# Naxaes/Rust-Swift-Raytracer

Measured on AMD Instinct MI355X. Metric: Mrays/sec + frames/sec at 1920×1080 spp=64; 1/2/4/8 MI355X, higher is better.
Workload: dtype f32; 1 GPU; c2: 1920x1080, spp 64, depth 8, 486 spheres, 0 triangles, COUNTER RNG; width=1920, height=1080, spp=64, depth=8, parallelism=one device renders the frame in place (no RCCL call)

## Files before the change

rust-swift-raytracer_amd/csrc/render.h:

```cpp
#pragma once

#include <hip/hip_runtime.h>

#include <cstdint>

#include "fastdiv.h"

namespace rtamd {

enum : uint32_t { kRngCounter = 1, kRngReplay = 2 };
enum : uint32_t { kRngSerialCount = 3, kRngSerialEstimate = 4, kRngSerialCheck = 5, kRngSerialCoalesce = 6,
                  kRngSerialPixel = 7 };
enum : uint32_t { kMatDiffuse = 0, kMatMetal = 1, kMatDielectric = 2, kMatEmission = 3 };
constexpr uint32_t kPrimaryTriStripW = 8;
#ifndef RT_TRACE_RING
#define RT_TRACE_RING 4
#endif
constexpr uint32_t kTraceRing = RT_TRACE_RING;
#ifdef RT_STAMPS
constexpr uint32_t kStatSlots = 24;
#else
constexpr uint32_t kStatSlots = 16;
#endif
constexpr uint32_t kStampSegs = 8;

struct SerialPred {
    const double *P;
    const double *mu;
    uint32_t spp, npix;
};
RT_HOST_DEVICE inline double serial_M(const SerialPred &m, uint32_t j) {
    const uint32_t p = j / m.spp;
    return p < m.npix ? m.P[p] + (double)(j - p * m.spp) * m.mu[p] : m.P[m.npix];
}

constexpr uint32_t kMaxJobParts = 1024;

struct TraceParams {
    const float4 *sph_hot;
    const float4 *sph_cold;
    const float4 *tri_hot;
    const float4 *tri_geo;
    const float *mats;
    float *samples;
    float *ring;
    uint32_t ring_shift;
    uint32_t *out;
    float inv_spp;
    uint32_t alpha_u8;
    uint32_t *job_counter;
    uint32_t *job_counter_next;
    unsigned long long *stats;
    const uint32_t *replay;
    float cam[12];
    float wden, hden;
    float wrcp, hrcp;
    uint32_t xdiv_uv;
    uint32_t nsph, nsph_padded, ntri;
    uint32_t width, height, spp;
    int32_t depth;
    uint32_t mode, seed;
    uint32_t row_block, rank, nranks;
    uint32_t slab_row0;
    uint32_t njobs;
    uint32_t npix;
    uint32_t chunk;
    uint32_t nparts;
    const float4 *bvh_nodes;
    const uint32_t *bvh_miss;
    const uint16_t *bvh_miss16;
    const float4 *bvh_prims;
    const uint32_t *bvh_prim_id;
    const float4 *big_hot;
    const uint32_t *big_id;
    uint32_t nnodes, nbig, nprims;
    uint32_t use_lds;
    uint32_t ablate;
    const float4 *sph_shade;
    const uint32_t *sph_kind;
    FastDiv div_spp, div_width, div_rowblock;
    uint32_t refill_min;
    uint32_t walk_min;
    uint32_t tri_walk_min;
    uint32_t steps;
    uint32_t step;
    float bvh_c[3], bvh_r, bvh_rmax, bvh_mag, bvh_inv_rmin;
    const uint4 *tbvh_nodes;
    const float4 *tbvh_tris;
    const uint32_t *tbvh_loose;
    uint32_t tnodes, ttris, tloose;
    float tbvh_c[3], tbvh_r, tbvh_mag;
    float tbvh_oc[3];
    float tq_base[3], tq_step[3], tq_nbase, tq_nstep;
    const uint4 *tw_nodes;
    uint32_t tw_depth;
    uint32_t wsteps;
    float cq_base[3], cq_step[3];
    const uint4 *cam_nodes;
    const float4 *cam_tris;
    uint32_t cam_nnodes;
    const uint32_t *ptl_off;
    const uint32_t *ptl_items;
    uint32_t ptl_spr;
    uint32_t ptl_always, ptl_end;
    const uint2 *spl;
    const uint32_t *win;
    SerialPred sM;
    const uint32_t *slo;
    const uint32_t *ctrl;
    uint32_t cbase;
    uint32_t nserial;
    uint32_t sspp;
    FastDiv div_sspp;
    uint32_t max_draws;
    uint32_t sL, sK;
    uint32_t gj32, gj_c0, gj_2p;
    const float4 *tw_tris;
    uint32_t tw_stride, tc_ncells;
    uint32_t tc_n[3];
    float tc_lo[3], tc_size, tc_inv_size;
    const uint4 *spix;
};

RT_HOST_DEVICE inline uint32_t serial_lo(const SerialPred &M, uint32_t a, uint32_t jl, uint32_t K,
                                         uint32_t depth, uint32_t nserial) {
    const uint32_t j = a + jl < nserial ? a + jl : nserial;
    double c = __builtin_floor(serial_M(M, j) - serial_M(M, a)) - (double)(K / 2u);
    const double hi = (double)depth * (double)jl;
    c = c < 0.0 ? 0.0 : c;
    c = c > hi ? hi : c;
    return (uint32_t)c;
}

hipError_t launch_trace(const TraceParams &p, uint32_t blocks, hipStream_t stream,
                        const uint4 *corner = nullptr);
hipError_t launch_sphere_lists(const float4 *prims, uint32_t n, const double *Mi, const double *o,
                               double e_abs, double wden, double hden, uint32_t width, uint32_t height,
                               int4 *rects, uint32_t *flag, uint2 *rec, hipStream_t stream);
size_t serial_tab_doubles(uint32_t npix);
hipError_t launch_serial_check_count(const float *flags, uint32_t n, unsigned long long *count,
                                     hipStream_t stream);
hipError_t launch_serial_moments(const float *est, uint32_t pix0, uint32_t n, uint32_t spp, uint32_t R,
                                 double scale, double *tab, uint32_t npix, hipStream_t stream);
hipError_t launch_serial_tables(double *tab, double *scratch, uint32_t npix, uint32_t spp, uint32_t L,
                                uint32_t n0, hipStream_t stream);
// ... 58 lines not shown
```

rust-swift-raytracer_amd/csrc/render.hip:

```cpp
#include <hip/hip_runtime.h>

#include <cstdint>
#include <type_traits>

#include "exactdiv.h"
#include "render.h"

#pragma clang fp contract(off)

namespace rtamd {
namespace {

struct F3 { float x, y, z; };

__device__ __forceinline__ F3 f3(float x, float y, float z) { return F3{x, y, z}; }
__device__ __forceinline__ F3 operator+(F3 a, F3 b) { return F3{a.x + b.x, a.y + b.y, a.z + b.z}; }
__device__ __forceinline__ F3 operator-(F3 a, F3 b) { return F3{a.x - b.x, a.y - b.y, a.z - b.z}; }
__device__ __forceinline__ F3 operator-(F3 a) { return F3{-a.x, -a.y, -a.z}; }
__device__ __forceinline__ F3 scale(F3 a, float s) { return F3{a.x * s, a.y * s, a.z * s}; }
__device__ __forceinline__ float dot(F3 a, F3 b) { return (a.x * b.x + a.y * b.y) + a.z * b.z; }
__device__ __forceinline__ F3 cross(F3 a, F3 b) {
    return F3{a.y * b.z - a.z * b.y, -(a.x * b.z - a.z * b.x), a.x * b.y - a.y * b.x};
}
__device__ __forceinline__ F3 divide_by(F3 a, float b) {
// ... 73 lines not shown
    return base[i];
#endif
}

__device__ __forceinline__ uint4 uniform_load_u4(const uint4 *base, uint32_t i) {
#if defined(__HIP_DEVICE_COMPILE__)
    typedef const __attribute__((address_space(4))) uint32_t *cu32_ptr;
    const cu32_ptr q = (cu32_ptr)(const void *)base + 4u * i;
    return make_uint4(q[0], q[1], q[2], q[3]);
#else
    return base[i];
#endif
}

__device__ __forceinline__ uint32_t fdiv(uint32_t n, const FastDiv &f) { return fastdiv_apply(n, f); }

constexpr uint32_t kWave = 64;
constexpr uint32_t kNodeEndDev = 0xFFFFFFFFu;
constexpr uint32_t kLeafBitDev = 0x80000000u;
constexpr uint32_t kSphListWalk = 0xFFFFu;
constexpr uint32_t kSphListMaxDev = 3u;
constexpr uint32_t kBatch = 8;

__device__ __forceinline__ void spheres_brute(const TraceParams &p, F3 org, F3 dir, float &best_t,
                                              int &best_i) {
    const float tmin = 0.001f;
#ifdef RT_BRUTE_PADDED
    const uint32_t n = p.nsph_padded;
#else
    const uint32_t n = p.nsph;
#endif
    for (uint32_t i0 = 0; i0 < n; i0 += kBatch) {
        const uint32_t m = n - i0;
        float hb[kBatch], disc[kBatch];
        bool any = false;
#pragma unroll
        for (uint32_t k = 0; k < kBatch; ++k) {
            hb[k] = 0.0f;
            disc[k] = -1.0f;
            if (k != 0u && k >= m) continue;
            const float4 S = uniform_load(p.sph_hot, i0 + k);
            const float ocx = org.x - S.x, ocy = org.y - S.y, ocz = org.z - S.z;
            hb[k] = (ocx * dir.x + ocy * dir.y) + ocz * dir.z;
            const float cc = ((ocx * ocx + ocy * ocy) + ocz * ocz) - S.w;
            disc[k] = hb[k] * hb[k] - cc;
            any |= disc[k] >= 0.0f;
        }
// ... 33 lines not shown
    const uint64_t kb = ((uint64_t)__float_as_uint(best_t) << 32) | (uint32_t)best_i;
    const bool take = valid && c != __builtin_inff() && kc < kb;
    if (take) { best_t = c; best_i = idx; }
    return take;
}

constexpr float kErrK = 3.0e-3f;

struct BvhView {
    const float4 *nodes;
    const uint32_t *miss32;
    const uint16_t *miss16;
    const float4 *prims;
    const uint32_t *ids;
    const float4 *shade;
    const uint32_t *kinds;
};

__device__ __forceinline__ float slab_rcp(float d) {
    return __builtin_amdgcn_fmed3f(__builtin_amdgcn_rcpf(d), -1e20f, 1e20f);
}

struct SphBound { float A, e_abs; };
__device__ __forceinline__ SphBound sph_bound(const TraceParams &p, F3 org) {
    const float ax = org.x - p.bvh_c[0], ay = org.y - p.bvh_c[1], az = org.z - p.bvh_c[2];
    return SphBound{__builtin_amdgcn_sqrtf((ax * ax + ay * ay) + az * az) * 1.00001f + p.bvh_r,
                    2e-6f * ((fabsf(org.x) + fabsf(org.y)) + fabsf(org.z) + p.bvh_mag)};
}
constexpr float kErrKq = 40.5f * 0x1p-24f;
__device__ __forceinline__ float sph_inflation(const TraceParams &p, SphBound b, float bt) {
    const float s = fminf(b.A, bt + p.bvh_rmax) * (1.0f + 3.0f * kErrK) + p.bvh_rmax;
    return fminf(kErrK * s, (kErrKq * s) * (s * p.bvh_inv_rmin)) + b.e_abs;
}

__device__ __forceinline__ void spheres_big(const TraceParams &p, F3 org, F3 dir, float &best_t,
                                            int &best_i) {
    for (uint32_t k = 0; k < p.nbig; ++k) {
        const float4 S = uniform_load(p.big_hot, k);
        sphere_candidate(S, org, dir, (int)uniform_load_u32(p.big_id, k), best_t, best_i);
    }
}

template <bool kLds>
__device__ __forceinline__ bool sphere_node(const BvhView &v, F3 inv, uint32_t ooff, float best_t, F3 nlo,
                                            F3 nhi, uint32_t &node, uint32_t &leaf, uint32_t &node_tests) {
    ++node_tests;
    float4 B0, B1;
    uint32_t miss, hit = 0;
    if (kLds) {
#if defined(__HIP_DEVICE_COMPILE__)
        typedef const __attribute__((address_space(3))) char *lds_cptr;
        const lds_cptr rec = (lds_cptr)(uintptr_t)node;
        B0 = *(const __attribute__((address_space(3))) float4 *)rec;
        B1 = *(const __attribute__((address_space(3))) float4 *)(rec + 16);
        const uint32_t lw = *(const __attribute__((address_space(3))) uint32_t *)(rec + 32 + ooff);
        hit = lw & 0xFFFFu;
        miss = lw >> 16;
#else
// ... 269 lines not shown
        const float omax = fmaxf(fmaxf(a, b), fmaxf(c, d));
        t0 = __builtin_fmaf(__builtin_fmaf(qlo, gs, omin), iv, c0);
        t1 = __builtin_fmaf(__builtin_fmaf(qhi, gs, omax), iv, c1);
    };
    float t0x, t1x, t0y, t1y, t0z, t1z;
    widen(lo16(w0), hi16(w1), nx0, nx1, nlo.x, nhi.x, gsx, inv.x, t0x, t1x);
    widen(hi16(w0), lo16(w2), ny0, ny1, nlo.y, nhi.y, gsy, inv.y, t0y, t1y);
    widen(lo16(w1), hi16(w2), nz0, nz1, nlo.z, nhi.z, gsz, inv.z, t0z, t1z);
    tn = fmaxf(fmaxf(fminf(t0x, t1x), fminf(t0y, t1y)), fminf(t0z, t1z));
    const float tf = fminf(fminf(fmaxf(t0x, t1x), fmaxf(t0y, t1y)), fmaxf(t0z, t1z));
    return !(tn > tf || tf < 0.001f || __float_as_int(tn) > __float_as_int(cap));
}

__device__ __forceinline__ void tri_leaf(const TraceParams &p, F3 org, F3 dir, bool cam,
                                         uint32_t leaf, float best_t, float &tri_t, int &tri_i,
                                         uint32_t &tri_in, uint32_t &tri_done, const float4 *wrecs = nullptr) {
    const float4 *recs = wrecs ? wrecs : cam ? p.cam_tris : p.tbvh_tris;
    const uint32_t first = leaf >> 3, end = first + (leaf & 7u);
    tri_done += leaf & 7u;
    for (uint32_t j = first; j < end; ++j)
        tri_record(recs + 4u * j, org, dir, best_t, tri_t, tri_i, tri_in);
}

template <bool kSerial>
__device__ __forceinline__ void job_pixel(const TraceParams &p, uint32_t job, uint32_t &s,
                                          uint32_t &col, uint32_t &row) {
    if (kSerial && p.mode == kRngSerialPixel) {
        const uint32_t pix = fdiv(p.cbase, p.div_sspp) + fdiv(job, p.div_spp);
        s = 0;
        row = fdiv(pix, p.div_width);
        col = pix - row * p.width;
        return;
    }
    if (kSerial) {
        const uint32_t jl = fdiv(job, p.div_spp);
        const uint32_t j = p.cbase + jl < p.nserial ? p.cbase + jl : p.nserial - 1u;
        const uint32_t pix = fdiv(j, p.div_sspp);
        s = j - pix * p.sspp;
        row = fdiv(pix, p.div_width);
        col = pix - row * p.width;
        return;
    }
    const uint32_t lp = fdiv(job, p.div_spp);
    s = job - lp * p.spp;
    const uint32_t q = fdiv(lp, p.div_width);
    col = lp - q * p.width;
    const uint32_t lr = p.slab_row0 + q;
    const uint32_t blk = fdiv(lr, p.div_rowblock);
    const uint32_t ir = (blk * p.nranks + p.rank) * p.row_block + (lr - blk * p.row_block);
    row = p.height - 1u - ir;
}

__device__ __forceinline__ void serial_pixel_span(const TraceParams &p, uint32_t q, uint32_t &plo,
                                                  uint32_t &phi) {
    if (p.spix != nullptr) {
        const uint4 s = p.spix[q];
        plo = s.x;
        phi = s.y;
        return;
    }
    const uint32_t a = p.cbase, ss = p.sspp;
    const uint32_t ln = min(p.sL, p.nserial - a);
    const uint32_t p0 = fdiv(a, p.div_sspp);
    const uint32_t jf = q == 0u ? 0u : (p0 + q) * ss - a;
    const uint32_t jz = min((p0 + q + 1u) * ss - a, ln) - 1u;
    plo = 2u * jf + 3u * p.slo[jf];
    phi = 2u * jz + 3u * (p.slo[jz] + p.sK - 1u);
}

__device__ __forceinline__ uint32_t serial_start(const TraceParams &p, uint32_t job) {
    const uint32_t jl = fdiv(job, p.div_spp);
    const uint32_t k = job - jl * p.spp;
    if (p.mode == kRngSerialCount)
// ... 11 lines not shown

__device__ __forceinline__ bool serial_pixel_job(const TraceParams &p, uint32_t job) {
    const uint32_t q = fdiv(job, p.div_spp);
    uint32_t plo, phi;
    serial_pixel_span(p, q, plo, phi);
    return plo + (job - q * p.spp) <= phi;
}

template <bool kSerial>
__device__ __forceinline__ void tri_primary_list(const TraceParams &p, uint32_t job, F3 org, F3 dir,
                                                 float best_t, float &tri_t, int &tri_i,
                                                 uint32_t &tri_in, uint32_t &tri_done) {
    uint32_t s, col, row;
    job_pixel<kSerial>(p, job, s, col, row);
    const uint32_t strip = row * p.ptl_spr + col / kPrimaryTriStripW;
    const uint32_t b = p.ptl_off[strip], e = p.ptl_off[strip + 1];
    tri_done += (e - b) + (p.ptl_end - p.ptl_always);
    for (uint32_t j = b; j < e; ++j)
        tri_record(p.cam_tris + 4u * p.ptl_items[j], org, dir, best_t, tri_t, tri_i, tri_in);
    for (uint32_t j = p.ptl_always; j < p.ptl_end; ++j)
        tri_record(p.cam_tris + 4u * p.ptl_items[j], org, dir, best_t, tri_t, tri_i, tri_in);
}

__device__ __forceinline__ uint32_t resolve_channel(const TraceParams &p, float sum) {
    return sat_u8(__builtin_sqrtf(sum * p.inv_spp) * 255.999f);
}
__device__ __forceinline__ void resolve_store_u8(const TraceParams &p, uint32_t lp, uint32_t R, uint32_t G,
                                                 uint32_t B) {
    const uint32_t q = fdiv(lp, p.div_width);
    const uint32_t col = lp - q * p.width;
    p.out[(size_t)(p.slab_row0 + q) * p.width + col] = R | (G << 8) | (B << 16) | (p.alpha_u8 << 24);
}
__device__ __forceinline__ void resolve_store(const TraceParams &p, uint32_t lp, float r, float g,
                                              float b) {
    resolve_store_u8(p, lp, resolve_channel(p, r), resolve_channel(p, g), resolve_channel(p, b));
}

#define RT_PLANE_LANES(mesh) ((mesh) < 2 || (mesh) == 3)
template <bool kPlaneLanes>
__device__ __forceinline__ void resolve_chunk(const TraceParams &p, const float *ring, uint32_t plane,
                                              uint32_t off, uint32_t base, uint32_t len,
                                              uint32_t lane) {
    __builtin_amdgcn_fence(__ATOMIC_RELEASE, "workgroup");
    __builtin_amdgcn_fence(__ATOMIC_ACQUIRE, "workgroup");
    const uint32_t spp = p.spp;
    const uint32_t np = fdiv(len, p.div_spp), pix0 = fdiv(base, p.div_spp);
    if (kPlaneLanes && 3u * np <= kWave && (spp & 3u) == 0) {
        const uint32_t c = lane >= np ? (lane >= 2u * np ? 2u : 1u) : 0u;
        const uint32_t g = lane - c * np;
        const bool on = lane < 3u * np;
        const float *src = ring + off + c * plane + (on ? g : 0u) * spp;
        float acc = 0.0f;
        for (uint32_t k = 0; k < spp; k += 16u) {
            float4 v[4];
#pragma unroll
            for (uint32_t q = 0; q < 4; ++q) {
                v[q] = make_float4(0.0f, 0.0f, 0.0f, 0.0f);
                if (on && k + 4u * q < spp) v[q] = *reinterpret_cast<const float4 *>(src + k + 4u * q);
            }
#pragma unroll
            for (uint32_t q = 0; q < 4; ++q) {
                if (k + 4u * q < spp) {
                    acc = acc + v[q].x;
                    acc = acc + v[q].y;
                    acc = acc + v[q].z;
                    acc = acc + v[q].w;
                }
            }
// ... 133 lines not shown
            const uint32_t ln = min(p.sL, p.nserial - p.cbase);
            const uint32_t p0 = fdiv(p.cbase, p.div_sspp);
            const uint32_t npq = E ? fdiv(p.cbase + ln - 1u, p.div_sspp) - p0 + 1u : 0u;
            p.spp = max(E, 1u);
            p.div_spp = make_fastdiv(p.spp);
            p.npix = npq;
            p.njobs = npq * E;
        }
    }
    if (!kSerial && p.job_counter_next != nullptr && blockIdx.x == 0)
        for (uint32_t i = threadIdx.x; i < kMaxJobParts; i += blockDim.x) p.job_counter_next[32u * i] = 0u;
    const uint32_t lane = __lane_id();
    auto kargs = [&]() -> const TraceParams & {
#if defined(__HIP_DEVICE_COMPILE__) && !defined(RT_NO_KARG_RELOAD)
        if (kSerial) return p;
        const __attribute__((address_space(4))) TraceParams *kp =
            (const __attribute__((address_space(4))) TraceParams *)__builtin_amdgcn_kernarg_segment_ptr();
        asm volatile("" : "+s"(kp));
        return *(const TraceParams *)kp;
#else
        return p;
#endif
    };
    extern __shared__ float4 lds[];
    BvhView view;
    const uint32_t sph_root = stage_tree<kLds, kCorner>(p, corner, lds, view);
    uint16_t *const tstack = reinterpret_cast<uint16_t *>(
                                 reinterpret_cast<char *>(lds) +
                                 (kLds ? (trace_tree_lds(p.nnodes, p.nprims, p.nsph_padded) + 15u) & ~(size_t)15u
                                       : 0u)) + threadIdx.x;
    uint32_t tsp = 0;

    F3 org = f3(0, 0, 0), dir = f3(0, 0, 0), inv = f3(0, 0, 0);
    float thr_r = 1.0f, thr_g = 1.0f, thr_b = 1.0f;
    uint32_t rng = 0, slot = ~0u, bounce = 0;
    uint32_t nscat = 0;
    uint32_t spl0 = 0, spl1 = kSphListWalk << 16;
    enum : uint32_t { kSetup = 0, kSph = 1, kTriInit = 2, kTri = 3, kShade = 4 };
    uint32_t phase = kSetup, node = 0, oct = 0;
    constexpr bool kWalkState = kMesh == 0 && !kStep;
    float best_t = 0.0f, tri_t = 0.0f, e = 0.0f;
    int best_i = -1, tri_i = -1;
    bool active = false;
    uint32_t rays = 0, tri_in = 0, sph_tests = 0, node_tests = 0, tnode_tests = 0,
             tri_done = 0;
    uint32_t it_all = 0, it_walk = 0, lanes_all = 0, lanes_walk = 0;
// ... 43 lines not shown
    } while (0)
#else
#define RT_STAMP(k) \
    do {            \
    } while (0)
#endif
    uint32_t part = (blockIdx.x * (blockDim.x / kWave) + threadIdx.x / kWave) % p.nparts;
    uint32_t tries = 0;
    auto part_begin = [&](uint32_t k) -> uint32_t {
        return (uint32_t)(((uint64_t)k * p.npix) / p.nparts) * p.spp;
    };
    uint32_t pbegin = part_begin(part), pend = part_begin(part + 1);
    uint32_t prefetch = 0;
    bool prefetch_pending = false;
    for (;;) {
        F3 vdir = dir;
        bool renorm = false;
        bool done = false;
        bool walked = false;
        const uint32_t nact = kCount ? (uint32_t)__popcll(__ballot(active)) : 0u;
        if (active) {
            float out_r = 0.0f, out_g = 0.0f, out_b = 0.0f;
            if (phase == kSetup) {
                const TraceParams &p = kargs();
                if ((int32_t)bounce >= p.depth) {
                    done = true;
                } else {
                    ++rays;
                    if (!kWalkState) {
                        inv = f3(slab_rcp(dir.x), slab_rcp(dir.y), slab_rcp(dir.z));
                        oct = (inv.x < 0.0f ? 1u : 0u) | (inv.y < 0.0f ? 2u : 0u) | (inv.z < 0.0f ? 4u : 0u);
                    }
                    best_t = __builtin_inff();
                    best_i = -1;
                    if (kBvh) {
                        spheres_big(p, org, dir, best_t, best_i);
                        if (!kWalkState)
                            node = kCorner ? sphere_corner_entry(sph_root, oct, p.nnodes)
                                           : sphere_walk_entry<kLds>(sph_root, oct, p.nnodes);
                        phase = (p.ablate & 1u) ? kTriInit : kSph;
                        if (!kMesh && bounce == 0 && (spl1 >> 16) != kSphListWalk) {
                            const uint32_t nc = spl1 >> 16;
                            sph_tests += nc;
                            if (nc > 0) sphere_candidate(view.prims[spl0 & 0xFFFFu], org, dir,
                                                         (int)view.ids[spl0 & 0xFFFFu], best_t, best_i);
                            if (nc > 1) sphere_candidate(view.prims[spl0 >> 16], org, dir,
                                                         (int)view.ids[spl0 >> 16], best_t, best_i);
                            if (nc > 2) sphere_candidate(view.prims[spl1 & 0xFFFFu], org, dir,
                                                         (int)view.ids[spl1 & 0xFFFFu], best_t, best_i);
                            phase = kTriInit;
                        }
                    } else {
                        spheres_brute(p, org, dir, best_t, best_i);
                        phase = kTriInit;
                    }
                }
            }
            RT_STAMP(1);
            uint32_t budget = p.steps;
            bool walk_now = true;
            if (!kMesh && p.walk_min != 0) {
                const uint32_t nwalk = (uint32_t)__popcll(__ballot(phase == kSph));
                const uint32_t nother = (uint32_t)__popcll(__ballot(phase != kSph && !done));
                walk_now = nwalk >= p.walk_min || nother == 0;
            }
            if (kBvh && phase == kSph && walk_now) {
                const TraceParams &p = kargs();
                walked = true;
                constexpr uint32_t kEnd = kLds ? 0xFFFFu : kNodeEndDev;
                const SphBound bnd = sph_bound(p, org);
                if (kWalkState) {
                    inv = f3(slab_rcp(dir.x), slab_rcp(dir.y), slab_rcp(dir.z));
                    oct = (inv.x < 0.0f ? 1u : 0u) | (inv.y < 0.0f ? 2u : 0u) | (inv.z < 0.0f ? 4u : 0u);
                    node = kCorner ? sphere_corner_entry(sph_root, oct, p.nnodes)
                                   : sphere_walk_entry<kLds>(sph_root, oct, p.nnodes);
                }
                if (kCorner) {
                    F3 nn, nf;
                    sphere_corner_slabs(org, inv, sph_inflation(p, bnd, best_t), oct, nn, nf);
                    const uint32_t offn = sph_root + 16u * oct, offf = sph_root + 112u - 16u * oct;
                    do {
                        uint32_t leaf;
                        if (sphere_node_corner(offn, offf, inv, best_t, nn, nf, node, leaf, node_tests))
                            sphere_leaf<true>(view, org, dir, leaf, best_t, best_i, sph_tests);
                    } while (node != 0xFFFFu && (!kStep || --budget != 0));
                } else {
                    F3 nlo, nhi;
                    sphere_slabs(org, inv, sph_inflation(p, bnd, best_t), nlo, nhi);
                    const uint32_t ooff = kLds ? 4u * oct : oct;
#ifdef RT_WALK_MIX
                    uint32_t wi = 0, wl = 0, wt = 0;
#endif
                    do {
                        uint32_t leaf;
                        const bool lf = sphere_node<kLds>(view, inv, ooff, best_t, nlo, nhi, node, leaf, node_tests);
#ifdef RT_WALK_MIX
                        if (kCount) {
                            ++wi;
// ... 260 lines not shown
            }
        }
        RT_STAMP(4);
        if (kCount && nact != 0) {
            const bool wk = __ballot(walked) != 0;
            ++it_all;
            lanes_all += nact;
            it_walk += wk ? 1u : 0u;
            lanes_walk += wk ? nact : 0u;
        }
        const uint64_t dead = __ballot(!active);
        const uint32_t ndead = (uint32_t)__popcll(dead);
        const bool refill = dead != 0 && (ndead >= p.refill_min || ndead == kWave);
        if (fused && refill) {
            const bool fin = !active && slot != ~0u;
            if (__ballot(fin) != 0) {
                const uint32_t lk = slot >> p.ring_shift;
#pragma unroll
                for (uint32_t k = 0; k < kTraceRing; ++k) {
                    if (rfree & (1u << k)) continue;
                    const uint32_t n = (uint32_t)__popcll(__ballot(fin && lk == k));
                    rleft[k] -= n;
                    if (n != 0 && rleft[k] == 0) {
                        const TraceParams &pc = kargs();
                        if (!(pc.ablate & 2u))
                            resolve_chunk<RT_PLANE_LANES(kMesh)>(pc, sbase, pstride, k << pc.ring_shift, rbase[k],
                                                  rlen[k], lane);
                        rfree |= 1u << k;
                    }
                }
                if (fin) slot = ~0u;
            }
        }
        RT_STAMP(5);
        if (refill && !exhausted && !(fused && rfree == 0 && pool_next >= pool_end)) {
            const TraceParams &pc = kargs();
            while (pool_next >= pool_end) {
                uint32_t base = 0;
                if (lane == 0) {
                    base = pbegin + (prefetch_pending ? prefetch
                                                      : atomicAdd(pc.job_counter + 32u * part, pc.chunk));
                    while (base >= pend && ++tries < pc.nparts) {
                        part = part + 1 == pc.nparts ? 0 : part + 1;
                        pbegin = part_begin(part);
                        pend = part_begin(part + 1);
                        base = pbegin + atomicAdd(pc.job_counter + 32u * part, pc.chunk);
                    }
                }
                prefetch_pending = false;
                base = __builtin_amdgcn_readfirstlane(base);
                part = __builtin_amdgcn_readfirstlane(part);
                tries = __builtin_amdgcn_readfirstlane(tries);
                pbegin = __builtin_amdgcn_readfirstlane(pbegin);
                pend = __builtin_amdgcn_readfirstlane(pend);
                if (base >= pend) {
                    exhausted = true;
#ifdef RT_WAVE_TIMES
                    wt_exh = __builtin_amdgcn_s_memrealtime();
#endif
// ... 23 lines not shown
#ifdef RT_WAVE_TIMES
                    wt_pull = __builtin_amdgcn_s_memrealtime();
                    wt_jobs_tail = pool_end - pool_next;
#endif
                    if (fused) {
                        const uint32_t k = (uint32_t)__builtin_ctz(rfree);
                        rfree &= ~(1u << k);
#pragma unroll
                        for (uint32_t i = 0; i < kTraceRing; ++i)
                            if (i == k) rbase[i] = base, rlen[i] = rleft[i] = pool_end - base;
                        cur_off = (k << pc.ring_shift) - base;
                    }
                }
                if (!kSerial) break;
            }
            const uint32_t avail = kSerial && exhausted ? 0u : pool_end - pool_next;
            const uint32_t rank = __builtin_amdgcn_mbcnt_hi(
                (uint32_t)(dead >> 32), __builtin_amdgcn_mbcnt_lo((uint32_t)dead, 0u));
            if (!active && rank < avail) {
                uint32_t job = pool_next + rank;
                if (kSerial && job >= gap_lo) job += gap_len;
                uint32_t s, col, row;
                uint64_t gjob = 0;
                if (!kSerial && pc.gj32) {
                    const uint32_t lp = fdiv(job, pc.div_spp);
                    const uint32_t q = fdiv(lp, pc.div_width);
                    col = lp - q * pc.width;
                    row = pc.height - 1u - (pc.slab_row0 + q);
                    gjob = job + pc.gj_c0 - q * pc.gj_2p;
                } else {
                    job_pixel<kSerial>(pc, job, s, col, row);
                    gjob = ((uint64_t)row * pc.width + col) * pc.spp + s;
                }
                slot = job + cur_off;
                bool take = true;
                if (kSerial) {
                    nscat = 0;
                    rng = serial_start(pc, job);
                    if (pc.mode == kRngSerialPixel) take = serial_pixel_job(pc, job);
                } else {
                    rng = (pc.mode == kRngReplay) ? pc.replay[gjob] : counter_seed(pc.seed, gjob);
                }
                const float un = draw_plus(rng, (float)col);
                const float vn = draw_plus(rng, (float)row);
#ifndef RT_NO_XDIV
                const bool xd = pc.xdiv_uv != 0;
#else
                const bool xd = false;
#endif
                const float u = xd ? xdiv(un, pc.wden, pc.wrcp) : un / pc.wden;
                const float v = xd ? xdiv(vn, pc.hden, pc.hrcp) : vn / pc.hden;
                const F3 h = f3(pc.cam[6], pc.cam[7], pc.cam[8]);
                const F3 vv = f3(pc.cam[9], pc.cam[10], pc.cam[11]);
                org = f3(pc.cam[0], pc.cam[1], pc.cam[2]);
                const F3 llc = f3(pc.cam[3], pc.cam[4], pc.cam[5]);
                vdir = ((llc + scale(h, u)) + scale(vv, v)) - org;
                renorm = true;
                if (kBvh && !kMesh && pc.spl != nullptr) {
                    if (pc.ablate & 4u) {
                        spl0 = 0;
                        spl1 = 0;
                    } else {
                        const uint2 r = pc.spl[(pc.height - 1u - row) * pc.width + col];
                        spl0 = r.x;
                        spl1 = r.y;
                    }
                }
                thr_r = thr_g = thr_b = 1.0f;
                bounce = 0;
                phase = kSetup;
                active = take;
            }
            pool_next += min(ndead, avail);
            if (!exhausted && !prefetch_pending && pool_end - pool_next < kWave) {
                if (lane == 0) prefetch = atomicAdd(p.job_counter + 32u * part, p.chunk);
                prefetch_pending = true;
            }
        }
        RT_STAMP(6);
        if (renorm) dir = unit(vdir);
        RT_STAMP(0);
        if (__ballot(active) == 0 && exhausted) break;
    }

    if (!kCount || p.stats == nullptr) return;
    uint64_t c[6] = {rays, tri_in, sph_tests, node_tests, tnode_tests, tri_done};
// ... 135 lines not shown
        hipLaunchKernelGGL((trace_kernel<false, false, kStep, kMesh, kCount, kSerial>), dim3(blocks),
                           dim3(256), trace_dyn_lds(p, false, kMesh == 3, 256), stream, p);
}

template <bool kCount, bool kSerial>
static void launch_trace_c(const TraceParams &p, uint32_t blocks, hipStream_t stream, const uint4 *corner) {
    const int mesh = trace_mesh_kind(p.ntri != 0, p.tnodes != 0);
    if (!kSerial && mesh == 2 && p.tw_nodes != nullptr) {
        if (p.step) launch_trace_t<true, 3, kCount, false>(p, blocks, stream, nullptr);
        else launch_trace_t<false, 3, kCount, false>(p, blocks, stream, nullptr);
        return;
    }
    if (p.step) {
        if (mesh == 2) launch_trace_t<true, 2, kCount, kSerial>(p, blocks, stream, corner);
        else if (mesh == 1) launch_trace_t<true, 1, kCount, kSerial>(p, blocks, stream, corner);
        else launch_trace_t<true, 0, kCount, kSerial>(p, blocks, stream, corner);
    } else {
        if (mesh == 2) launch_trace_t<false, 2, kCount, kSerial>(p, blocks, stream, corner);
        else if (mesh == 1) launch_trace_t<false, 1, kCount, kSerial>(p, blocks, stream, corner);
        else launch_trace_t<false, 0, kCount, kSerial>(p, blocks, stream, corner);
    }
}

hipError_t launch_trace(const TraceParams &p, uint32_t blocks, hipStream_t stream, const uint4 *corner) {
    if (p.mode >= kRngSerialCount) launch_trace_c<false, true>(p, blocks, stream, nullptr);
    else if (p.stats) launch_trace_c<true, false>(p, blocks, stream, corner);
    else launch_trace_c<false, false>(p, blocks, stream, corner);
    return hipGetLastError();
}

hipError_t launch_resolve_ex(const float *samples, uint32_t *out, uint32_t npix, uint32_t spp,
                             float inv_spp, uint32_t width, uint32_t slab_row0,
                             hipStream_t stream) {
    const uint32_t per_block = kResolveWaves * kWave;
    const uint32_t blocks = (npix + per_block - 1) / per_block;
    hipLaunchKernelGGL(resolve_kernel, dim3(blocks), dim3(per_block), 0, stream, samples, out, npix,
                       spp, inv_spp, width, slab_row0);
    return hipGetLastError();
}

template <bool kStep, int kMesh, bool kCount, bool kSerial>
static hipError_t trace_occupancy_t(int *blocks_per_cu, int variant, size_t lds_bytes) {
    constexpr int kind = kSerial ? 2 : kCount ? 1 : 0;
    if constexpr (kMesh == 0 && !kSerial) {
        if (variant == 3)
            return hipOccupancyMaxActiveBlocksPerMultiprocessor(
                blocks_per_cu, corner::trace_kernel<true, true, kStep, 0, kCount, false>,
// ... 784 lines not shown
static void launch_coalesce_m(const TraceParams &p, uint32_t *path, uint32_t *bend, uint32_t L, uint32_t Kmax,
                              uint32_t R, size_t tree_bytes, size_t lds, unsigned long long *dbg,
                              hipStream_t stream) {
    const uint32_t nb = (L + R - 1) / R;
    const int mesh = trace_mesh_kind(p.ntri != 0, p.tnodes != 0);
    if (mesh == 2)
        hipLaunchKernelGGL((serial_coalesce_kernel<kBvh, kLds, 2>), dim3(nb), dim3(kCoalesceThreads), lds, stream, p,
                           path, bend, L, Kmax, R, (uint32_t)tree_bytes, dbg);
    else if (mesh == 1)
        hipLaunchKernelGGL((serial_coalesce_kernel<kBvh, kLds, 1>), dim3(nb), dim3(kCoalesceThreads), lds, stream, p,
                           path, bend, L, Kmax, R, (uint32_t)tree_bytes, dbg);
    else
        hipLaunchKernelGGL((serial_coalesce_kernel<kBvh, kLds, 0>), dim3(nb), dim3(kCoalesceThreads), lds, stream, p,
                           path, bend, L, Kmax, R, (uint32_t)tree_bytes, dbg);
}

size_t serial_coalesce_search_lds(uint32_t K, uint32_t depth) { return coalesce_lds_bytes(K, depth); }

size_t serial_coalesce_lds(const TraceParams &p, uint32_t K, bool tree_lds) {
    const size_t tb = tree_lds ? (trace_lds_bytes(p) + 15) & ~(size_t)15 : 0;
    return tb + coalesce_lds_bytes(K, p.depth > 0 ? (uint32_t)p.depth : 0u);
}

hipError_t launch_serial_coalesce(const TraceParams &p, uint32_t *path, uint32_t *bend, uint32_t L, uint32_t Kmax,
                                  uint32_t R, bool tree_lds, unsigned long long *dbg, hipStream_t stream) {
    if (!L || !R) return hipSuccess;
    const size_t tb = tree_lds ? (trace_lds_bytes(p) + 15) & ~(size_t)15 : 0;
    const size_t lds = serial_coalesce_lds(p, Kmax, tree_lds);
    if (p.nnodes && tree_lds) launch_coalesce_m<true, true>(p, path, bend, L, Kmax, R, tb, lds, dbg, stream);
    else if (p.nnodes) launch_coalesce_m<true, false>(p, path, bend, L, Kmax, R, tb, lds, dbg, stream);
    else launch_coalesce_m<false, false>(p, path, bend, L, Kmax, R, tb, lds, dbg, stream);
    return hipGetLastError();
}

__global__ __launch_bounds__(256) void serial_moments_kernel(const float *__restrict__ est, uint32_t pix0,
                                                             uint32_t n, uint32_t spp, uint32_t R,
                                                             double scale, double *__restrict__ tab,
                                                             uint32_t npix) {
    const uint32_t i = blockIdx.x * blockDim.x + threadIdx.x;
    if (i >= n) return;
    const uint32_t per = spp * R;
    const float *src = est + (size_t)i * per;
    double s = 0.0, sq = 0.0;
    bool bad = false;
    for (uint32_t k = 0; k < per; ++k) {
        const float b = src[k];
        bad |= !(b >= 0.0f);
        s += (double)b;
        sq += (double)b * (double)b;
// ... 442 lines not shown
```

Baseline: 65590 Mrays/s.

## Group kernel arguments into 64-byte blocks loaded with single scalar loads

Reorders TraceParams into 64-byte-aligned sub-structs, one per kernel phase (setup, walk, shade, resolve, refill), and reloads each phase's fields from the kernarg segment with one s_load_dwordx8/x16, pinned in SGPRs via an empty asm. Derived fields (walk_nnodes, rf_flags) are precomputed on the host so fewer distinct fields are read. The aim is to cut scalar-register pressure and scattered kernarg loads in the persistent trace loop. The cost is a more rigid layout guarded by static_asserts, and possibly extra SGPRs live while a block is held.

Measured after the change: 65570 Mrays/s. Within noise of the previous version (-0.0%).

```diff
diff --git a/rust-swift-raytracer_amd/csrc/render.h b/rust-swift-raytracer_amd/csrc/render.h
--- a/rust-swift-raytracer_amd/csrc/render.h
+++ b/rust-swift-raytracer_amd/csrc/render.h
@@ -2,6 +2,7 @@
 
 #include <hip/hip_runtime.h>
 
+#include <cstddef>
 #include <cstdint>
 
 #include "fastdiv.h"
@@ -36,74 +37,123 @@
 
 constexpr uint32_t kMaxJobParts = 1024;
 
-struct TraceParams {
+
+struct alignas(64) SetupParams {
+    const float4 *big_hot;
+    const uint32_t *big_id;
     const float4 *sph_hot;
-    const float4 *sph_cold;
+    int32_t depth;
+    uint32_t nbig;
+    uint32_t nnodes;
+    uint32_t ablate;
+    uint32_t nsph, nsph_padded;
+};
+struct alignas(64) WalkParams {
+    float bvh_c[3], bvh_r, bvh_rmax, bvh_mag, bvh_inv_rmin;
+    uint32_t walk_nnodes;
+};
+struct alignas(64) TriSetupParams {
+    const uint32_t *tbvh_loose;
     const float4 *tri_hot;
+    const float4 *tbvh_tris;
+    const float4 *cam_tris;
+    const uint32_t *ptl_off;
+    const uint32_t *ptl_items;
+    uint32_t tloose, ttris, cam_nnodes, ntri;
+};
+struct alignas(64) TriSetup2Params {
+    float tbvh_c[3], tbvh_r, tbvh_mag;
+    uint32_t ptl_spr;
+    uint32_t ptl_always, ptl_end;
+    uint32_t tnodes;
+};
+struct alignas(64) TriWalkParams {
+    const uint4 *tbvh_nodes;
+    const uint4 *cam_nodes;
+    float tbvh_oc[3];
+    float tq_base[3], tq_step[3], tq_nbase, tq_nstep;
+};
+struct alignas(64) TriWalk2Params {
+    float cq_base[3], cq_step[3];
+};
+struct alignas(64) TriWideParams {
+    const uint4 *tw_nodes;
+    const float4 *tw_tris;
+    uint32_t tw_stride, tc_ncells;
+    uint32_t wsteps;
+    uint32_t tw_depth;
+    uint32_t tc_n[3];
+    float tc_lo[3], tc_size, tc_inv_size;
+};
+struct alignas(64) ShadeParams {
+    const float4 *sph_shade;
+    const uint32_t *sph_kind;
     const float4 *tri_geo;
     const float *mats;
-    float *samples;
-    float *ring;
-    uint32_t ring_shift;
+};
+struct alignas(64) ResolveParams {
     uint32_t *out;
     float inv_spp;
     uint32_t alpha_u8;
+    uint32_t ring_shift;
+};
+enum : uint32_t {
+    kRfGj32 = 1,
+    kRfReplay = 2,
+    kRfXdiv = 4,
+    kRfSpl = 8,
+    kRfNoResolve = 16,
+    kRfNoSplLoad = 32
+};
+struct alignas(64) RefillJobParams {
+    const uint32_t *replay;
+    FastDiv div_spp, div_width;
+    uint32_t rf_flags;
+    uint32_t slab_row0;
+    uint32_t height, seed;
+    uint32_t gj_c0, gj_2p;
+};
+struct alignas(64) RefillCamParams {
+    float cam[12];
+    float wden, hden;
+    float wrcp, hrcp;
+};
+struct alignas(64) RefillTileParams {
+    const uint2 *spl;
+    FastDiv div_rowblock;
+    uint32_t rank, nranks;
+};
+
+struct TraceParams : SetupParams, WalkParams, TriSetupParams, TriSetup2Params, TriWalkParams, TriWalk2Params,
+                     TriWideParams, ShadeParams, ResolveParams, RefillJobParams, RefillCamParams,
+                     RefillTileParams {
+    const float4 *sph_cold;
+    float *samples;
+    float *ring;
     uint32_t *job_counter;
     uint32_t *job_counter_next;
     unsigned long long *stats;
-    const uint32_t *replay;
-    float cam[12];
-    float wden, hden;
-    float wrcp, hrcp;
-    uint32_t xdiv_uv;
-    uint32_t nsph, nsph_padded, ntri;
-    uint32_t width, height, spp;
-    int32_t depth;
-    uint32_t mode, seed;
-    uint32_t row_block, rank, nranks;
-    uint32_t slab_row0;
+    uint32_t width, spp;
+    uint32_t row_block;
     uint32_t njobs;
     uint32_t npix;
     uint32_t chunk;
     uint32_t nparts;
+    uint32_t refill_min;
+    uint32_t walk_min;
+    uint32_t tri_walk_min;
+    uint32_t steps;
+    uint32_t step;
+    uint32_t mode;
+    uint32_t xdiv_uv;
+    uint32_t gj32;
     const float4 *bvh_nodes;
     const uint32_t *bvh_miss;
     const uint16_t *bvh_miss16;
     const float4 *bvh_prims;
     const uint32_t *bvh_prim_id;
-    const float4 *big_hot;
-    const uint32_t *big_id;
-    uint32_t nnodes, nbig, nprims;
+    uint32_t nprims;
     uint32_t use_lds;
-    uint32_t ablate;
-    const float4 *sph_shade;
-    const uint32_t *sph_kind;
-    FastDiv div_spp, div_width, div_rowblock;
-    uint32_t refill_min;
-    uint32_t walk_min;
-    uint32_t tri_walk_min;
-    uint32_t steps;
-    uint32_t step;
-    float bvh_c[3], bvh_r, bvh_rmax, bvh_mag, bvh_inv_rmin;
-    const uint4 *tbvh_nodes;
-    const float4 *tbvh_tris;
-    const uint32_t *tbvh_loose;
-    uint32_t tnodes, ttris, tloose;
-    float tbvh_c[3], tbvh_r, tbvh_mag;
-    float tbvh_oc[3];
-    float tq_base[3], tq_step[3], tq_nbase, tq_nstep;
-    const uint4 *tw_nodes;
-    uint32_t tw_depth;
-    uint32_t wsteps;
-    float cq_base[3], cq_step[3];
-    const uint4 *cam_nodes;
-    const float4 *cam_tris;
-    uint32_t cam_nnodes;
-    const uint32_t *ptl_off;
-    const uint32_t *ptl_items;
-    uint32_t ptl_spr;
-    uint32_t ptl_always, ptl_end;
-    const uint2 *spl;
     const uint32_t *win;
     SerialPred sM;
     const uint32_t *slo;
@@ -114,13 +164,51 @@
     FastDiv div_sspp;
     uint32_t max_draws;
     uint32_t sL, sK;
-    uint32_t gj32, gj_c0, gj_2p;
-    const float4 *tw_tris;
-    uint32_t tw_stride, tc_ncells;
-    uint32_t tc_n[3];
-    float tc_lo[3], tc_size, tc_inv_size;
     const uint4 *spix;
 };
+
+#define RT_BLOCK_CHECK(B, used_dwords)                                                               \
+    static_assert(sizeof(B) == 64 && alignof(B) == 64, #B ": one 64-B block");                      \
+    static_assert(used_dwords <= 16, #B ": at most 16 dwords")
+RT_BLOCK_CHECK(SetupParams, 12);
+RT_BLOCK_CHECK(WalkParams, 8);
+RT_BLOCK_CHECK(TriSetupParams, 16);
+RT_BLOCK_CHECK(TriSetup2Params, 9);
+RT_BLOCK_CHECK(TriWalkParams, 15);
+RT_BLOCK_CHECK(TriWalk2Params, 6);
+RT_BLOCK_CHECK(TriWideParams, 16);
+RT_BLOCK_CHECK(ShadeParams, 8);
+RT_BLOCK_CHECK(ResolveParams, 5);
+RT_BLOCK_CHECK(RefillJobParams, 16);
+RT_BLOCK_CHECK(RefillCamParams, 16);
+RT_BLOCK_CHECK(RefillTileParams, 8);
+#undef RT_BLOCK_CHECK
+static_assert(offsetof(SetupParams, nsph_padded) == 44 && offsetof(WalkParams, walk_nnodes) == 28 &&
+                  offsetof(TriSetupParams, ntri) == 60 && offsetof(TriSetup2Params, tnodes) == 32 &&
+                  offsetof(TriWalkParams, tq_nstep) == 56 && offsetof(TriWideParams, tc_inv_size) == 60 &&
+                  offsetof(ShadeParams, mats) == 24 && offsetof(ResolveParams, ring_shift) == 16 &&
+                  offsetof(RefillJobParams, gj_2p) == 60 && offsetof(RefillCamParams, hrcp) == 60 &&
+                  offsetof(RefillTileParams, nranks) == 28,
+              "section blocks: the fields the section loads cover (render.hip block loads)");
+#pragma GCC diagnostic push
+#pragma GCC diagnostic ignored "-Winvalid-offsetof"
+static_assert(offsetof(TraceParams, big_hot) == 0 && offsetof(TraceParams, bvh_c) == 64 &&
+                  offsetof(TraceParams, tbvh_loose) == 128 && offsetof(TraceParams, tbvh_c) == 192 &&
+                  offsetof(TraceParams, tbvh_nodes) == 256 && offsetof(TraceParams, cq_base) == 320 &&
+                  offsetof(TraceParams, tw_nodes) == 384 && offsetof(TraceParams, sph_shade) == 448 &&
+                  offsetof(TraceParams, out) == 512 && offsetof(TraceParams, replay) == 576 &&
+                  offsetof(TraceParams, cam) == 640 && offsetof(TraceParams, spl) == 704 &&
+                  offsetof(TraceParams, sph_cold) == 768,
+              "TraceParams: the section blocks in order, 64 B each");
+#pragma GCC diagnostic pop
+static_assert(alignof(TraceParams) == 64 && sizeof(TraceParams) % 64 == 0, "TraceParams: 64-B blocks");
+
+inline void trace_params_finish(TraceParams &p) {
+    p.walk_nnodes = p.nnodes;
+    p.rf_flags = (p.gj32 ? kRfGj32 : 0u) | (p.mode == kRngReplay ? kRfReplay : 0u) | (p.xdiv_uv ? kRfXdiv : 0u) |
+                 (p.spl != nullptr ? kRfSpl : 0u) | ((p.ablate & 2u) ? kRfNoResolve : 0u) |
+                 ((p.ablate & 4u) ? kRfNoSplLoad : 0u);
+}
 
 RT_HOST_DEVICE inline uint32_t serial_lo(const SerialPred &M, uint32_t a, uint32_t jl, uint32_t K,
                                          uint32_t depth, uint32_t nserial) {
diff --git a/rust-swift-raytracer_amd/csrc/render.hip b/rust-swift-raytracer_amd/csrc/render.hip
--- a/rust-swift-raytracer_amd/csrc/render.hip
+++ b/rust-swift-raytracer_amd/csrc/render.hip
@@ -119,7 +119,8 @@
 constexpr uint32_t kSphListMaxDev = 3u;
 constexpr uint32_t kBatch = 8;
 
-__device__ __forceinline__ void spheres_brute(const TraceParams &p, F3 org, F3 dir, float &best_t,
+template <class P>
+__device__ __forceinline__ void spheres_brute(const P &p, F3 org, F3 dir, float &best_t,
                                               int &best_i) {
     const float tmin = 0.001f;
 #ifdef RT_BRUTE_PADDED
@@ -199,18 +200,21 @@
 }
 
 struct SphBound { float A, e_abs; };
-__device__ __forceinline__ SphBound sph_bound(const TraceParams &p, F3 org) {
+template <class P>
+__device__ __forceinline__ SphBound sph_bound(const P &p, F3 org) {
     const float ax = org.x - p.bvh_c[0], ay = org.y - p.bvh_c[1], az = org.z - p.bvh_c[2];
     return SphBound{__builtin_amdgcn_sqrtf((ax * ax + ay * ay) + az * az) * 1.00001f + p.bvh_r,
                     2e-6f * ((fabsf(org.x) + fabsf(org.y)) + fabsf(org.z) + p.bvh_mag)};
 }
 constexpr float kErrKq = 40.5f * 0x1p-24f;
-__device__ __forceinline__ float sph_inflation(const TraceParams &p, SphBound b, float bt) {
+template <class P>
+__device__ __forceinline__ float sph_inflation(const P &p, SphBound b, float bt) {
     const float s = fminf(b.A, bt + p.bvh_rmax) * (1.0f + 3.0f * kErrK) + p.bvh_rmax;
     return fminf(kErrK * s, (kErrKq * s) * (s * p.bvh_inv_rmin)) + b.e_abs;
 }
 
-__device__ __forceinline__ void spheres_big(const TraceParams &p, F3 org, F3 dir, float &best_t,
+template <class P>
+__device__ __forceinline__ void spheres_big(const P &p, F3 org, F3 dir, float &best_t,
                                             int &best_i) {
     for (uint32_t k = 0; k < p.nbig; ++k) {
         const float4 S = uniform_load(p.big_hot, k);
@@ -526,33 +530,33 @@
         tri_record(recs + 4u * j, org, dir, best_t, tri_t, tri_i, tri_in);
 }
 
-template <bool kSerial>
-__device__ __forceinline__ void job_pixel(const TraceParams &p, uint32_t job, uint32_t &s,
+template <bool kSerial, class P>
+__device__ __forceinline__ void job_pixel(const P &p, uint32_t job, uint32_t &s,
                                           uint32_t &col, uint32_t &row) {
-    if (kSerial && p.mode == kRngSerialPixel) {
-        const uint32_t pix = fdiv(p.cbase, p.div_sspp) + fdiv(job, p.div_spp);
-        s = 0;
-        row = fdiv(pix, p.div_width);
-        col = pix - row * p.width;
-        return;
-    }
-    if (kSerial) {
+    if constexpr (kSerial) {
+        if (p.mode == kRngSerialPixel) {
+            const uint32_t pix = fdiv(p.cbase, p.div_sspp) + fdiv(job, p.div_spp);
+            s = 0;
+            row = fdiv(pix, p.div_width);
+            col = pix - row * p.width;
+            return;
+        }
         const uint32_t jl = fdiv(job, p.div_spp);
         const uint32_t j = p.cbase + jl < p.nserial ? p.cbase + jl : p.nserial - 1u;
         const uint32_t pix = fdiv(j, p.div_sspp);
         s = j - pix * p.sspp;
         row = fdiv(pix, p.div_width);
         col = pix - row * p.width;
-        return;
-    }
-    const uint32_t lp = fdiv(job, p.div_spp);
-    s = job - lp * p.spp;
-    const uint32_t q = fdiv(lp, p.div_width);
-    col = lp - q * p.width;
-    const uint32_t lr = p.slab_row0 + q;
-    const uint32_t blk = fdiv(lr, p.div_rowblock);
-    const uint32_t ir = (blk * p.nranks + p.rank) * p.row_block + (lr - blk * p.row_block);
-    row = p.height - 1u - ir;
+    } else {
+        const uint32_t lp = fdiv(job, p.div_spp);
+        s = job - lp * p.div_spp.d;
+        const uint32_t q = fdiv(lp, p.div_width);
+        col = lp - q * p.div_width.d;
+        const uint32_t lr = p.slab_row0 + q;
+        const uint32_t blk = fdiv(lr, p.div_rowblock);
+        const uint32_t ir = (blk * p.nranks + p.rank) * p.div_rowblock.d + (lr - blk * p.div_rowblock.d);
+        row = p.height - 1u - ir;
+    }
 }
 
 __device__ __forceinline__ void serial_pixel_span(const TraceParams &p, uint32_t q, uint32_t &plo,
@@ -610,28 +614,31 @@
         tri_record(p.cam_tris + 4u * p.ptl_items[j], org, dir, best_t, tri_t, tri_i, tri_in);
 }
 
-__device__ __forceinline__ uint32_t resolve_channel(const TraceParams &p, float sum) {
+template <class P>
+__device__ __forceinline__ uint32_t resolve_channel(const P &p, float sum) {
     return sat_u8(__builtin_sqrtf(sum * p.inv_spp) * 255.999f);
 }
-__device__ __forceinline__ void resolve_store_u8(const TraceParams &p, uint32_t lp, uint32_t R, uint32_t G,
+template <class P>
+__device__ __forceinline__ void resolve_store_u8(const P &p, uint32_t lp, uint32_t R, uint32_t G,
                                                  uint32_t B) {
     const uint32_t q = fdiv(lp, p.div_width);
-    const uint32_t col = lp - q * p.width;
-    p.out[(size_t)(p.slab_row0 + q) * p.width + col] = R | (G << 8) | (B << 16) | (p.alpha_u8 << 24);
-}
-__device__ __forceinline__ void resolve_store(const TraceParams &p, uint32_t lp, float r, float g,
+    const uint32_t col = lp - q * p.div_width.d;
+    p.out[(size_t)(p.slab_row0 + q) * p.div_width.d + col] = R | (G << 8) | (B << 16) | (p.alpha_u8 << 24);
+}
+template <class P>
+__device__ __forceinline__ void resolve_store(const P &p, uint32_t lp, float r, float g,
                                               float b) {
     resolve_store_u8(p, lp, resolve_channel(p, r), resolve_channel(p, g), resolve_channel(p, b));
 }
 
 #define RT_PLANE_LANES(mesh) ((mesh) < 2 || (mesh) == 3)
-template <bool kPlaneLanes>
-__device__ __forceinline__ void resolve_chunk(const TraceParams &p, const float *ring, uint32_t plane,
+template <bool kPlaneLanes, class P>
+__device__ __forceinline__ void resolve_chunk(const P &p, const float *ring, uint32_t plane,
                                               uint32_t off, uint32_t base, uint32_t len,
                                               uint32_t lane) {
     __builtin_amdgcn_fence(__ATOMIC_RELEASE, "workgroup");
     __builtin_amdgcn_fence(__ATOMIC_ACQUIRE, "workgroup");
-    const uint32_t spp = p.spp;
+    const uint32_t spp = p.div_spp.d;
     const uint32_t np = fdiv(len, p.div_spp), pix0 = fdiv(base, p.div_spp);
     if (kPlaneLanes && 3u * np <= kWave && (spp & 3u) == 0) {
         const uint32_t c = lane >= np ? (lane >= 2u * np ? 2u : 1u) : 0u;
@@ -811,6 +818,34 @@
         return p;
 #endif
     };
+    auto section_load = [&](auto tag, auto ndw) {
+        typedef decltype(tag) B;
+        constexpr int N = decltype(ndw)::value;
+        static_assert(N == 8 || N == 16, "one s_load_dwordx8 or x16");
+        const TraceParams &kp = kargs();
+#if defined(__HIP_DEVICE_COMPILE__) && !defined(RT_NO_KARG_RELOAD)
+        if constexpr (!kSerial) {
+            typedef uint32_t dwords __attribute__((ext_vector_type(N)));
+            return *(const __attribute__((address_space(4))) dwords *)(const void *)static_cast<const B *>(&kp);
+        } else {
+            return B(static_cast<const B &>(kp));
+        }
+#else
+        return B(static_cast<const B &>(kp));
+#endif
+    };
+    auto section_use = [&](auto tag, auto v) {
+        typedef decltype(tag) B;
+        if constexpr (std::is_same<decltype(v), B>::value) {
+            return v;
+        } else {
+            asm volatile("" : "+s"(v));
+            B b;
+            __builtin_memcpy((void *)&b, &v, sizeof(v));
+            return b;
+        }
+    };
+#define RT_SECTION_BLOCK(B, N) section_use(B{}, section_load(B{}, std::integral_constant<int, N>{}))
     extern __shared__ float4 lds[];
     BvhView view;
     const uint32_t sph_root = stage_tree<kLds, kCorner>(p, corner, lds, view);
@@ -900,7 +935,7 @@
         if (active) {
             float out_r = 0.0f, out_g = 0.0f, out_b = 0.0f;
             if (phase == kSetup) {
-                const TraceParams &p = kargs();
+                const SetupParams p = RT_SECTION_BLOCK(SetupParams, 16);
                 if ((int32_t)bounce >= p.depth) {
                     done = true;
                 } else {
@@ -943,15 +978,15 @@
                 walk_now = nwalk >= p.walk_min || nother == 0;
             }
             if (kBvh && phase == kSph && walk_now) {
-                const TraceParams &p = kargs();
+                const WalkParams p = RT_SECTION_BLOCK(WalkParams, 8);
                 walked = true;
                 constexpr uint32_t kEnd = kLds ? 0xFFFFu : kNodeEndDev;
                 const SphBound bnd = sph_bound(p, org);
                 if (kWalkState) {
                     inv = f3(slab_rcp(dir.x), slab_rcp(dir.y), slab_rcp(dir.z));
                     oct = (inv.x < 0.0f ? 1u : 0u) | (inv.y < 0.0f ? 2u : 0u) | (inv.z < 0.0f ? 4u : 0u);
-                    node = kCorner ? sphere_corner_entry(sph_root, oct, p.nnodes)
-                                   : sphere_walk_entry<kLds>(sph_root, oct, p.nnodes);
+                    node = kCorner ? sphere_corner_entry(sph_root, oct, p.walk_nnodes)
+                                   : sphere_walk_entry<kLds>(sph_root, oct, p.walk_nnodes);
                 }
                 if (kCorner) {
                     F3 nn, nf;
@@ -1258,8 +1293,11 @@
                     const uint32_t n = (uint32_t)__popcll(__ballot(fin && lk == k));
                     rleft[k] -= n;
                     if (n != 0 && rleft[k] == 0) {
-                        const TraceParams &pc = kargs();
-                        if (!(pc.ablate & 2u))
+                        struct ResolveView : ResolveParams, RefillJobParams {};
+                        const auto rdw = section_load(ResolveParams{}, std::integral_constant<int, 8>{});
+                        const auto jdw = section_load(RefillJobParams{}, std::integral_constant<int, 16>{});
+                        const ResolveView pc{section_use(ResolveParams{}, rdw), section_use(RefillJobParams{}, jdw)};
+                        if (!(pc.rf_flags & kRfNoResolve))
                             resolve_chunk<RT_PLANE_LANES(kMesh)>(pc, sbase, pstride, k << pc.ring_shift, rbase[k],
                                                   rlen[k], lane);
                         rfree |= 1u << k;
@@ -1271,6 +1309,10 @@
         RT_STAMP(5);
         if (refill && !exhausted && !(fused && rfree == 0 && pool_next >= pool_end)) {
             const TraceParams &pc = kargs();
+            struct RefillView : RefillJobParams, RefillTileParams {};
+            const auto jdw = section_load(RefillJobParams{}, std::integral_constant<int, 16>{});
+            const auto tdw = section_load(RefillTileParams{}, std::integral_constant<int, 8>{});
+            const RefillView rv{section_use(RefillJobParams{}, jdw), section_use(RefillTileParams{}, tdw)};
             while (pool_next >= pool_end) {
                 uint32_t base = 0;
                 if (lane == 0) {
@@ -1340,15 +1382,16 @@
                 if (kSerial && job >= gap_lo) job += gap_len;
                 uint32_t s, col, row;
                 uint64_t gjob = 0;
-                if (!kSerial && pc.gj32) {
-                    const uint32_t lp = fdiv(job, pc.div_spp);
-                    const uint32_t q = fdiv(lp, pc.div_width);
-                    col = lp - q * pc.width;
-                    row = pc.height - 1u - (pc.slab_row0 + q);
-                    gjob = job + pc.gj_c0 - q * pc.gj_2p;
+                if (!kSerial && (rv.rf_flags & kRfGj32)) {
+                    const uint32_t lp = fdiv(job, rv.div_spp);
+                    const uint32_t q = fdiv(lp, rv.div_width);
+                    col = lp - q * rv.div_width.d;
+                    row = rv.height - 1u - (rv.slab_row0 + q);
+                    gjob = job + rv.gj_c0 - q * rv.gj_2p;
                 } else {
-                    job_pixel<kSerial>(pc, job, s, col, row);
-                    gjob = ((uint64_t)row * pc.width + col) * pc.spp + s;
+                    if constexpr (kSerial) job_pixel<true>(pc, job, s, col, row);
+                    else job_pixel<false>(rv, job, s, col, row);
+                    gjob = ((uint64_t)row * rv.div_width.d + col) * rv.div_spp.d + s;
                 }
                 slot = job + cur_off;
                 bool take = true;
@@ -1357,29 +1400,31 @@
                     rng = serial_start(pc, job);
                     if (pc.mode == kRngSerialPixel) take = serial_pixel_job(pc, job);
                 } else {
-                    rng = (pc.mode == kRngReplay) ? pc.replay[gjob] : counter_seed(pc.seed, gjob);
+                    rng = (rv.rf_flags & kRfReplay) ? rv.replay[gjob] : counter_seed(rv.seed, gjob);
                 }
+                const auto cam_dwords = section_load(RefillCamParams{}, std::integral_constant<int, 16>{});
                 const float un = draw_plus(rng, (float)col);
                 const float vn = draw_plus(rng, (float)row);
+                const RefillCamParams rc = section_use(RefillCamParams{}, cam_dwords);
 #ifndef RT_NO_XDIV
-                const bool xd = pc.xdiv_uv != 0;
+                const bool xd = (rv.rf_flags & kRfXdiv) != 0;
 #else
                 const bool xd = false;
 #endif
-                const float u = xd ? xdiv(un, pc.wden, pc.wrcp) : un / pc.wden;
-                const float v = xd ? xdiv(vn, pc.hden, pc.hrcp) : vn / pc.hden;
-                const F3 h = f3(pc.cam[6], pc.cam[7], pc.cam[8]);
-                const F3 vv = f3(pc.cam[9], pc.cam[10], pc.cam[11]);
-                org = f3(pc.cam[0], pc.cam[1], pc.cam[2]);
-                const F3 llc = f3(pc.cam[3], pc.cam[4], pc.cam[5]);
+                const float u = xd ? xdiv(un, rc.wden, rc.wrcp) : un / rc.wden;
+                const float v = xd ? xdiv(vn, rc.hden, rc.hrcp) : vn / rc.hden;
+                const F3 h = f3(rc.cam[6], rc.cam[7], rc.cam[8]);
+                const F3 vv = f3(rc.cam[9], rc.cam[10], rc.cam[11]);
+                org = f3(rc.cam[0], rc.cam[1], rc.cam[2]);
+                const F3 llc = f3(rc.cam[3], rc.cam[4], rc.cam[5]);
                 vdir = ((llc + scale(h, u)) + scale(vv, v)) - org;
                 renorm = true;
-                if (kBvh && !kMesh && pc.spl != nullptr) {
-                    if (pc.ablate & 4u) {
+                if (kBvh && !kMesh && (rv.rf_flags & kRfSpl)) {
+                    if (rv.rf_flags & kRfNoSplLoad) {
                         spl0 = 0;
                         spl1 = 0;
                     } else {
-                        const uint2 r = pc.spl[(pc.height - 1u - row) * pc.width + col];
+                        const uint2 r = rv.spl[(rv.height - 1u - row) * rv.div_width.d + col];
                         spl0 = r.x;
                         spl1 = r.y;
                     }
@@ -1561,7 +1606,9 @@
     }
 }
 
-hipError_t launch_trace(const TraceParams &p, uint32_t blocks, hipStream_t stream, const uint4 *corner) {
+hipError_t launch_trace(const TraceParams &params, uint32_t blocks, hipStream_t stream, const uint4 *corner) {
+    TraceParams p = params;
+    trace_params_finish(p);
     if (p.mode >= kRngSerialCount) launch_trace_c<false, true>(p, blocks, stream, nullptr);
     else if (p.stats) launch_trace_c<true, false>(p, blocks, stream, corner);
     else launch_trace_c<false, false>(p, blocks, stream, corner);
@@ -2392,9 +2439,11 @@
     return tb + coalesce_lds_bytes(K, p.depth > 0 ? (uint32_t)p.depth : 0u);
 }
 
-hipError_t launch_serial_coalesce(const TraceParams &p, uint32_t *path, uint32_t *bend, uint32_t L, uint32_t Kmax,
+hipError_t launch_serial_coalesce(const TraceParams &params, uint32_t *path, uint32_t *bend, uint32_t L, uint32_t Kmax,
                                   uint32_t R, bool tree_lds, unsigned long long *dbg, hipStream_t stream) {
     if (!L || !R) return hipSuccess;
+    TraceParams p = params;
+    trace_params_finish(p);
     const size_t tb = tree_lds ? (trace_lds_bytes(p) + 15) & ~(size_t)15 : 0;
     const size_t lds = serial_coalesce_lds(p, Kmax, tree_lds);
     if (p.nnodes && tree_lds) launch_coalesce_m<true, true>(p, path, bend, L, Kmax, R, tb, lds, dbg, stream);
```
